# yanyan-li/Structure-SLAM-PointLine

Hardware: AMD Instinct MI355X
Metric: front-end frames/sec (ORB+LSD extract+match) 640x480 @1000kp/200ln (higher is better)
Workload: dtype u8

## Files before the change

include/sslam_frontend.h:

```cpp
#ifndef SSLAM_FRONTEND_H
#define SSLAM_FRONTEND_H

#include <stddef.h>
#include <stdint.h>

#ifdef __cplusplus
extern "C" {
#endif

#define SSLAM_OK 0
#define SSLAM_ERR_INVALID (-1)
#define SSLAM_ERR_NO_DEVICE (-2)
#define SSLAM_ERR_CAPACITY (-3)
#define SSLAM_ERR_HIP (-4)
#define SSLAM_ERR_UNSUPPORTED (-5)

typedef struct sslam_keypoint {
    float x, y, size, angle, response;
    int32_t octave, class_id;
} sslam_keypoint;

typedef struct sslam_keyline {
    float angle;
    int32_t class_id, octave;
// ... 185 lines not shown
int sslam_undistort_keypoints_batch_dev(sslam_ctx* ctx, const sslam_camera* cam, const sslam_keypoint* d_kp, const int32_t* d_counts,
                                        int nframes, int cap, sslam_keypoint* d_kp_un, void* stream);
int sslam_orb_set_camera(sslam_orb* orb, const sslam_camera* cam);
int sslam_frontend_batch_match_camera(sslam_orb* orb, sslam_lines* lines, const sslam_camera* cam, const uint8_t* images, int n, int w, int h,
                                      size_t stride, size_t image_stride, int chunk, sslam_keypoint* kp_out, sslam_keypoint* kpun_out,
                                      uint8_t* desc_out, int32_t* nkp_out, int cap, sslam_keyline* kl_out, uint8_t* ldesc_out,
                                      double* linefn_out, int32_t* nl_out, int lcap, const sslam_batch_match* match);

enum { SSLAM_PIX_GRAY = 0, SSLAM_PIX_RGB = 1, SSLAM_PIX_BGR = 2, SSLAM_PIX_RGBA = 3, SSLAM_PIX_BGRA = 4 };
int sslam_gray_from_color(sslam_ctx* ctx, int format, const uint8_t* img, int w, int h, size_t stride, uint8_t* gray, size_t gray_stride);
int sslam_gray_from_color_batch_dev(sslam_ctx* ctx, int format, const uint8_t* d_src, int w, int h, size_t pitch, size_t image_stride, int nframes,
                                    uint8_t* d_gray, size_t gray_pitch, size_t gray_image_stride, void* stream);
int sslam_frontend_batch_color(sslam_orb* orb, sslam_lines* lines, const sslam_camera* cam, int format, const uint8_t* images, int n, int w, int h,
                               size_t stride, size_t image_stride, int chunk, sslam_keypoint* kp_out, sslam_keypoint* kpun_out, uint8_t* desc_out,
                               int32_t* nkp_out, int cap, sslam_keyline* kl_out, uint8_t* ldesc_out, double* linefn_out, int32_t* nl_out, int lcap,
                               const sslam_batch_match* match);

typedef struct sslam_group sslam_group;
#define SSLAM_GROUP_ID_BYTES 128
typedef struct sslam_record_header { int32_t n_kp, n_ln, frame, bytes; } sslam_record_header;
typedef struct sslam_frontend_params {
    int32_t nfeatures; float scale_factor; int32_t nlevels, ini_th_fast, min_th_fast, max_lines;
} sslam_frontend_params;

int sslam_group_create(int ngpu, sslam_group** out);
int sslam_group_unique_id(uint8_t id_out[SSLAM_GROUP_ID_BYTES]);
int sslam_group_create_rank(int device, int rank, int nranks, const uint8_t id[SSLAM_GROUP_ID_BYTES], sslam_group** out);
int sslam_group_destroy(sslam_group* group);
int sslam_group_size(const sslam_group* group);
int sslam_group_rank(const sslam_group* group);

int sslam_pack_records_dev(sslam_ctx* ctx, int nframes, int frame0, int frame_step,
                           const sslam_keypoint* d_kp, const uint8_t* d_desc, const int32_t* d_nkp, int cap,
                           const sslam_keyline* d_kl, const uint8_t* d_ldesc, const double* d_linefn, const int32_t* d_nl, int lcap,
                           uint8_t* d_out, uint64_t out_capacity, uint64_t* d_total_bytes, void* stream);
uint64_t sslam_record_stream_capacity(int nframes, int cap, int lcap);
int sslam_unpack_records(const uint8_t* stream, uint64_t bytes, int nframes,
                         sslam_keypoint* kp_out, uint8_t* desc_out, int32_t* nkp_out, int cap,
                         sslam_keyline* kl_out, uint8_t* ldesc_out, double* linefn_out, int32_t* nl_out, int lcap, int* nrecords_out);

int sslam_group_gather_dev(sslam_group* group, const uint8_t* d_send, const uint64_t* d_send_bytes,
                           uint8_t* d_recv, uint64_t recv_capacity, uint64_t* bytes_per_rank_out, void* stream);

int sslam_frontend_batch_sharded(sslam_group* group, const sslam_frontend_params* params,
                                 const uint8_t* images, int n, int w, int h, size_t stride, size_t image_stride,
                                 sslam_keypoint* kp_out, uint8_t* desc_out, int32_t* nkp_out, int cap,
                                 sslam_keyline* kl_out, uint8_t* ldesc_out, double* linefn_out, int32_t* nl_out, int lcap);
int sslam_shard_layout(int n, int ngpu, int* chunk_slots_out, int* nchunks_out);
int sslam_shard_frame(int n, int ngpu, int chunk, int gpu, int slot);
int sslam_shard_chunk_count(int n, int ngpu, int chunk, int gpu);

int sslam_lines_debug_segments(sslam_lines* ln, int frame, float* seg_out, int cap, int* n_out);
int sslam_lines_debug_cycles(sslam_lines* ln, int frame, long long* out8);
#ifdef __cplusplus
}
#endif
#endif
```

structure-slam-pointline_amd/csrc/lines.hip:

```cpp
#include "common.h"
#include <cmath>
#include <cstdlib>
#include <cfloat>
#include <algorithm>

namespace sslam { int launch_nfa_stream(sslam_ctx* ctx, hipStream_t st, uint8_t* ws, const void* plan, size_t planBytes, const double* lgam, uint8_t* clArea, size_t clFrameBytes,
                                        size_t stageOff, int nframes, int waves, long long spinTicks, bool besideCore); }
namespace sslam { int launch_nfa_stage(sslam_ctx* ctx, hipStream_t st, uint8_t* ws, const void* plan, size_t planBytes, const double* lgam, int nframes); }

using namespace sslam;

namespace {

#include "lsd_plan.h"
#include "lsd_front.h"
#include "lsd_regions.h"
#include "lsd_cluster.h"
#include "lsd_nfa.h"
#include "lbd.h"

__global__ void k_zero_misc(uint8_t* ws, LsdPlan P) {
    Misc* m = (Misc*)(ws + (size_t)blockIdx.x * P.frameBytes + P.offMisc);
    if (threadIdx.x == 0) {
        m->maxS = 0; m->nDefined = 0; m->nSeg = 0; m->nCand = 0; m->nKl = 0; m->overflow = 0; m->claim = 0;
#if defined(SSLAM_LSD_DRIFT_VERIFY) || defined(SSLAM_LSD_CYCLES)
        m->cyc[5] = 0; m->cyc[6] = 0; m->cyc[7] = 0;
#endif
    }
}

__global__ __launch_bounds__(256) void k_lines_status(const uint8_t* __restrict__ ws, LsdPlan P, int nframes, int maxLines, int cap, int* __restrict__ status) {
    __shared__ int cnt[2], first[2];
    if (threadIdx.x < 2) { cnt[threadIdx.x] = 0; first[threadIdx.x] = 0x7FFFFFFF; }
    __syncthreads();
    for (int b = threadIdx.x; b < nframes; b += 256) {
        const Misc* m = (const Misc*)(ws + (size_t)b * P.frameBytes + P.offMisc);
        if (min(m->nSeg, maxLines) > cap) { atomicAdd(&cnt[0], 1); atomicMin(&first[0], b); }
        if (m->overflow) { atomicAdd(&cnt[1], 1); atomicMin(&first[1], b); }
    }
    __syncthreads();
    if (threadIdx.x == 0) { status[0] = cnt[0]; status[1] = first[0]; status[2] = cnt[1]; status[3] = first[1]; }
}

}

struct sslam_lines {
    sslam_ctx* ctx;
    int maxLines;
    int planW = 0, planH = 0;
    LsdPlan plan;
    DevBuf dWs, dTabs, dTaps, dLgam, dGtab;
    size_t clFrame = 0; int clSlots = 0;
    DevBuf dCl;
    int wsFrames = 0, lastFrames = 0;
    hipEvent_t coreEvent = nullptr;
    hipEvent_t coreWait = nullptr, coreDone = nullptr;
    int lastN = -1;
    DevBuf dImg, dKl, dDesc, dFn, dCounts;
    HostPinned hOut;
    bool constsUploaded = false;
    int blurVariant = 0;
    int nfaVariant = 1, lbdBitOrder = 1, lsdResize = 0;
    int seedOrder = 0;
    int sMin = 0;
    bool fusedGeometry = false;
    hipStream_t nfaStream = nullptr; hipEvent_t nfaFork = nullptr, nfaJoin = nullptr;
};

static std::vector<int> taps_q8(int n, double sigma) {
    std::vector<double> k(n);
    double sum = 0, s2 = -0.5 / (sigma * sigma);
    for (int i = 0; i < n; ++i) { double x = i - (n - 1) * 0.5; k[i] = std::exp(s2 * x * x); sum += k[i]; }
    std::vector<int> t(n);
    double err = 0; long isum = 0;
    for (int i = 0; i < n / 2; ++i) {
        double adj = k[i] / sum * 256.0 + err;
        int v = (int)lrint(adj);
        err = adj - v; t[i] = t[n - 1 - i] = v; isum += v;
    }
// ... 484 lines not shown
    std::lock_guard<std::recursive_mutex> lk(L->ctx->mu);
    int rc;
    if ((rc = L->dCounts.ensure(16))) return rc;
    hipStream_t st = stream_ ? (hipStream_t)stream_ : L->ctx->stream;
    if ((rc = sslam_lines_batch_status_dev(L, cap, L->dCounts.as<int32_t>(), st))) return rc;
    int h[4] = {0, 0, 0, 0};
    SSLAM_HIP(hipMemcpyAsync(h, L->dCounts.p, sizeof(h), hipMemcpyDeviceToHost, st));
    SSLAM_HIP(hipStreamSynchronize(st));
    if (truncated_frames_out) *truncated_frames_out = h[0];
    if (unsupported_frames_out) *unsupported_frames_out = h[2];
    if (first_frame_out) *first_frame_out = h[2] ? h[3] : h[0] ? h[1] : -1;
    if (h[2]) { set_error("sslam_lines_batch_status: %d frame(s) with more than %d candidate rectangles (first: frame %d)", h[2], MAX_SEG, h[3]); return SSLAM_ERR_UNSUPPORTED; }
    if (h[0]) { set_error("sslam_lines_batch_status: %d frame(s) hold more lines than the capacity %d (first: frame %d)", h[0], cap, h[1]); return SSLAM_ERR_CAPACITY; }
    return SSLAM_OK;
}

extern "C" int sslam_lines_debug_segments(sslam_lines* L, int frame, float* seg_out, int cap, int* n_out) {
    if (!L || frame < 0 || frame >= L->lastFrames || !n_out) return SSLAM_ERR_INVALID;
    SSLAM_HIP(hipSetDevice(L->ctx->device));
    SSLAM_HIP(hipStreamSynchronize(L->ctx->stream));
    const LsdPlan& P = L->plan;
    const uint8_t* base = L->dWs.as<uint8_t>() + (size_t)frame * P.frameBytes;
    Misc m;
    SSLAM_HIP(hipMemcpy(&m, base + P.offMisc, sizeof(m), hipMemcpyDeviceToHost));
    *n_out = m.nSeg;
    int n = std::min(m.nSeg, cap);
    if (n > 0 && seg_out) SSLAM_HIP(hipMemcpy(seg_out, base + P.offSeg, sizeof(float) * 4 * (size_t)n, hipMemcpyDeviceToHost));
    return SSLAM_OK;
}

extern "C" int sslam_lines_set_core_event(sslam_lines* L, void* hip_event) {
    if (!L) return SSLAM_ERR_INVALID;
    L->coreEvent = (hipEvent_t)hip_event;
    return SSLAM_OK;
}

extern "C" int sslam_lines_set_core_gate(sslam_lines* L, void* wait_event, void* done_event) {
    if (!L) return SSLAM_ERR_INVALID;
    L->coreWait = (hipEvent_t)wait_event; L->coreDone = (hipEvent_t)done_event;
    return SSLAM_OK;
}

extern "C" int sslam_lines_debug_cycles(sslam_lines* L, int frame, long long* out8) {
    if (!L || frame < 0 || frame >= L->lastFrames || !out8) return SSLAM_ERR_INVALID;
    SSLAM_HIP(hipSetDevice(L->ctx->device));
    SSLAM_HIP(hipDeviceSynchronize());
    const LsdPlan& P = L->plan;
    Misc m;
    SSLAM_HIP(hipMemcpy(&m, L->dWs.as<uint8_t>() + (size_t)frame * P.frameBytes + P.offMisc, sizeof(m), hipMemcpyDeviceToHost));
    for (int i = 0; i < 8; ++i) out8[i] = m.cyc[i];
    return SSLAM_OK;
}

#ifdef SSLAM_TESTING
extern "C" int sslam_lines_debug_cluster(sslam_lines* L, int frame, long long* out8) {
    if (!L || frame < 0 || frame >= L->clSlots || !out8 || !L->dCl.p || !L->clFrame) return SSLAM_ERR_INVALID;
    SSLAM_HIP(hipSetDevice(L->ctx->device));
    SSLAM_HIP(hipDeviceSynchronize());
    ClCtl c;
    SSLAM_HIP(hipMemcpy(&c, L->dCl.as<uint8_t>() + (size_t)frame * L->clFrame, sizeof(c), hipMemcpyDeviceToHost));
    for (int i = 0; i < 8; ++i) out8[i] = c.stat[i];
    return SSLAM_OK;
}

namespace {
struct ScopedDev {
    void* p = nullptr;
    ~ScopedDev() { if (p) (void)hipFree(p); }
};
}

extern "C" int sslam_selftest_exact_div(sslam_ctx* ctx, int n, long long pairs, long long* mismatches_out) {
    if (!ctx || n < 3 || pairs <= 0 || !mismatches_out) return SSLAM_ERR_INVALID;
    SSLAM_HIP(hipSetDevice(ctx->device));
    ScopedDev tabMem, badMem;
    SSLAM_HIP(hipMalloc(&tabMem.p, sizeof(double) * (2 * (size_t)n + 48)));
    SSLAM_HIP(hipMalloc(&badMem.p, sizeof(unsigned long long)));
    double* tab = (double*)tabMem.p; unsigned long long* bad = (unsigned long long*)badMem.p;
    SSLAM_HIP(hipMemset(bad, 0, sizeof(unsigned long long)));
    { const int rc = upload_nfa_tables(tab, n, ctx->stream); if (rc) return rc; }
    const int threads = 256 * 1024, iters = (int)((pairs + threads - 1) / threads);
    hipLaunchKernelGGL(k_selftest_div, dim3(1024), dim3(256), 0, ctx->stream, tab + n + 48, n, 0x1234567ull, iters, bad);
    unsigned long long h = 0;
    SSLAM_HIP(hipMemcpyAsync(&h, bad, sizeof(h), hipMemcpyDeviceToHost, ctx->stream));
    SSLAM_HIP(hipStreamSynchronize(ctx->stream));
    *mismatches_out = (long long)h;
    return SSLAM_OK;
}

extern "C" int sslam_selftest_tail_test(sslam_ctx* ctx, long long samples, long long* disagree_out, long long* ambiguous_out) {
    if (!ctx || samples <= 0 || !disagree_out || !ambiguous_out) return SSLAM_ERR_INVALID;
    SSLAM_HIP(hipSetDevice(ctx->device));
    ScopedDev dMem;
    SSLAM_HIP(hipMalloc(&dMem.p, 2 * sizeof(unsigned long long)));
    unsigned long long* d = (unsigned long long*)dMem.p;
    SSLAM_HIP(hipMemset(d, 0, 2 * sizeof(unsigned long long)));
    const int threads = 256 * 1024, iters = (int)((samples + threads - 1) / threads);
    const double logNT = 5 * (std::log10(512.0) + std::log10(384.0)) / 2 + std::log10(11.0);
    hipLaunchKernelGGL(k_selftest_tail, dim3(1024), dim3(256), 0, ctx->stream, 0xABCDEF12345ull, iters, logNT, d);
    unsigned long long h[2] = {0, 0};
    SSLAM_HIP(hipMemcpyAsync(h, d, sizeof(h), hipMemcpyDeviceToHost, ctx->stream));
    SSLAM_HIP(hipStreamSynchronize(ctx->stream));
    *disagree_out = (long long)h[0]; *ambiguous_out = (long long)h[1];
    return SSLAM_OK;
}

// ... 191 lines not shown
```

structure-slam-pointline_amd/csrc/lsd_plan.h:

```cpp
#pragma once

constexpr double kPI = 3.14159265358979323846;
constexpr double DEG2RAD = kPI / 180;
constexpr double M_3_2_PI_ = (3 * kPI) / 2, M_2PI_ = 2 * kPI;
constexpr float NOTDEF_F = -1024.0f;
constexpr int CS_SHIFT = 3, S_SHIFT = 2;
constexpr unsigned USED_BIT = 0x80000000u;
constexpr int N_BINS = 1024;
#ifndef SSLAM_TILE_PX
#define SSLAM_TILE_PX 8192
#endif
constexpr int TILE_PX = SSLAM_TILE_PX;
constexpr int MAX_SEG = 8192;
constexpr int NUM_BANDS = 9, BAND_W = 7, LSP_H = 63;

struct LsdPlan {
    int w, h;
    int sw, sh, spitch;
    int npx;
    int nTiles, tileRows;
    int nXB;
    int sMin;
    size_t frameBytes;
    int tW, cW;
    size_t offBlur, offT, offS, offCs, offCand, offFlag, offNfa, offOrder, offTileHist, offReg, offSeg, offMisc, offDxy, offKl, offSortIdx, offSegCnt, offComp, offSorted, offLbdDir;
    int blurTaps[7];
    int blur5Taps[5];
    int tabX, tabY;
    double rho, prec, p, logNT;
    int minRegSize;
    int nfaVariant;
    int lbdBitOrder;
    int lsdResize;
};

struct Misc {
    int maxS;
    int nDefined;
    int nSeg;
    int nCand;
    int nKl;
    int overflow;
    int claim;
    int pad_;
    long long cyc[8];
};

struct NfaStreamCtl {
    int candReady;
    int candFinal;
    int claim;
    int expired;
};
constexpr int NFA_STREAM_BLOCK = 8;
constexpr int NFA_STREAM_CTL_OFF = 256;

__device__ __forceinline__ int tix(int x, int y, int tW) { return y * tW + x; }
__device__ __forceinline__ int cix(int x, int y, int cW) { return y * cW + x; }

struct RectD { double x1, y1, x2, y2, width, x, y, theta, dx, dy, prec, p; };

#ifndef SSLAM_LSD_QCAP
#define SSLAM_LSD_QCAP 768
#endif
constexpr int QCAP = SSLAM_LSD_QCAP;
constexpr int MAXC = 5;

__device__ __forceinline__ double angle_diff_signed(double a, double b) {
    double diff = a - b;
    while (diff <= -kPI) diff += M_2PI_;
    while (diff > kPI) diff -= M_2PI_;
    return diff;
}
__device__ __forceinline__ bool is_aligned_val(float aDeg, double theta, double prec) {
    double n_theta = fabs(theta - (double)aDeg * DEG2RAD);
    const double wrapped = fabs(n_theta - M_2PI_);
    n_theta = n_theta > M_3_2_PI_ ? wrapped : n_theta;
    return aDeg != NOTDEF_F && n_theta <= prec;
}
```

structure-slam-pointline_amd/csrc/lsd_regions.h:

```cpp
#pragma once

struct RegQ {
    unsigned* lds; unsigned* glb;
    __device__ __forceinline__ unsigned get(int i) const { return i < QCAP ? lds[i] : glb[i]; }
    __device__ __forceinline__ unsigned get_n(int i, int n) const {
        if (n <= QCAP) { unsigned v = lds[i]; asm volatile("" : "+v"(v)); return v; }
        return get(i);
    }
    __device__ __forceinline__ void set(int i, unsigned v) const { if (i < QCAP) lds[i] = v; else glb[i] = v; }
};
struct Planes {
    float* T; const float2* Cs; const int* S; int tW, cW;
    __device__ __forceinline__ unsigned* Tb() const { return (unsigned*)T; }
    __device__ __forceinline__ float ldT(int i) const { return *(const float*)((const char*)T + ((unsigned)i << 2)); }
    __device__ __forceinline__ void stT(int i, float v) const { *(float*)((char*)T + ((unsigned)i << 2)) = v; }
    __device__ __forceinline__ float2 ldCs(int i) const { return *(const float2*)((const char*)Cs + ((unsigned)i << CS_SHIFT)); }
    __device__ __forceinline__ int ti(int x, int y) const { return (int)(__umul24((unsigned)y, (unsigned)tW) + (unsigned)x); }
    __device__ __forceinline__ int ti(unsigned e) const { return (int)(__umul24(e >> 16, (unsigned)tW) + (e & 0xFFFFu)); }

};
__device__ __forceinline__ bool t_free(float t) { return __float_as_int(t) >= 0; }
__device__ __forceinline__ float t_used(float t) { return __int_as_float(__float_as_int(t) | (int)USED_BIT); }
constexpr int MW_BM_WORDS = 256 * 256 / 32, MW_REACH = 126;
__device__ __forceinline__ int mw_bit(int x, int y) { return ((y & 255) << 8) | (x & 255); }
// ... 12 lines not shown
__device__ __forceinline__ double readlane_d(double v, int l) {
    int lo = __builtin_amdgcn_readlane(__double2loint(v), l), hi = __builtin_amdgcn_readlane(__double2hiint(v), l);
    return __hiloint2double(hi, lo);
}

__device__ __forceinline__ float div_unit_range(float a, float b) {
    float r = __builtin_amdgcn_rcpf(b);
    r = __builtin_fmaf(__builtin_fmaf(-b, r, 1.0f), r, r);
    float q = a * r;
    q = __builtin_fmaf(__builtin_fmaf(-b, q, a), r, q);
    return __builtin_fmaf(__builtin_fmaf(-b, q, a), r, q);
}

__device__ __forceinline__ float fast_atan2_deg_unit(float y, float x) {
    const float p1 = 0.9997878412794807f * (float)(180 / 3.14159265358979323846);
    const float p3 = -0.3258083974640975f * (float)(180 / 3.14159265358979323846);
    const float p5 = 0.1555786518463281f * (float)(180 / 3.14159265358979323846);
    const float p7 = -0.04432655554792128f * (float)(180 / 3.14159265358979323846);
    const float eps = (float)2.2204460492503131e-16;
    const float ax = fabsf(x), ay = fabsf(y);
    const float c = div_unit_range(fminf(ax, ay), __fadd_rn(fmaxf(ax, ay), eps));
    const float c2 = __fmul_rn(c, c);
    float a = __fmul_rn(__fadd_rn(__fmul_rn(__fadd_rn(__fmul_rn(__fadd_rn(__fmul_rn(p7, c2), p5), c2), p3), c2), p1), c);
    if (ax < ay) a = __fsub_rn(90.f, a);
    a = fabsf(__fsub_rn(__int_as_float((__float_as_int(x) >> 31) & 0x43340000), a));
    a = fabsf(__fsub_rn(__int_as_float((__float_as_int(y) >> 31) & 0x43b40000), a));
    return a;
}

#ifdef SSLAM_TESTING
__global__ void k_selftest_region_div(unsigned long long seed, int iters, unsigned long long* __restrict__ out) {
    unsigned long long x = seed + (blockIdx.x * (unsigned long long)blockDim.x + threadIdx.x) * 0x9E3779B97F4A7C15ull;
    auto rnd = [&]() { x ^= x << 13; x ^= x >> 7; x ^= x << 17; return (float)((double)(x >> 11) * 0x1p-53); };
    unsigned long long bad = 0, bad2 = 0;
    for (int it = 0; it < iters; ++it) {
        const float ex = exp2f(-54.f + 74.f * rnd()), ey = exp2f(-54.f + 74.f * rnd());
        float sx = (1.f + rnd()) * ex, sy = (1.f + rnd()) * ey;
        const int mode = (int)(rnd() * 16.f);
        if (mode == 0) sy = 0.f; else if (mode == 1) sx = sy; else if (mode == 2) sx = 6.123234e-17f * (float)(1 + (int)(rnd() * 4000.f));
        else if (mode == 3) { sx = (float)(int)(rnd() * 100000.f); sy = (float)(int)(rnd() * 100000.f); if (sx == 0.f && sy == 0.f) sx = 1.f; }
        if ((x & 1) && sx != 0.f) sx = -sx;
        if ((x & 2) && sy != 0.f) sy = -sy;
        if (sx == 0.f && sy == 0.f) continue;
        const float eps = (float)2.2204460492503131e-16;
        const float ax = fabsf(sx), ay = fabsf(sy), mn = fminf(ax, ay), mx = __fadd_rn(fmaxf(ax, ay), eps);
        if (__float_as_int(div_unit_range(mn, mx)) != __float_as_int(__fdiv_rn(mn, mx))) ++bad;
        if (__float_as_int(fast_atan2_deg_unit(sy, sx)) != __float_as_int(fast_atan2_deg<false>(sy, sx))) ++bad2;
    }
    if (bad) atomicAdd(out, bad);
    if (bad2) atomicAdd(out + 1, bad2);
}
#endif

#ifndef SSLAM_LSD_DRIFT
#define SSLAM_LSD_DRIFT 1
#endif
template <bool LAT, bool WIDE, int MARK = MARK_MAP, class G = TorusHelper>
__device__ int region_grow_w(int seedX, int seedY, float seedDeg, float seedCos, float seedSin, int sw, int sh, const Planes& pl, const RegQ& rq,
                             double prec, double& regAngleOut, long long* __restrict__ verifyCnt, unsigned* __restrict__ bm = nullptr, int capN = 0) {
#ifndef SSLAM_LSD_READLANE
#define SSLAM_LSD_READLANE 0
#endif
    static_assert(MARK == MARK_MAP || LAT, "private marks are written by the lone-wave flavour only");
    constexpr bool RL = LAT || SSLAM_LSD_READLANE;
    constexpr bool DRIFT = !WIDE && SSLAM_LSD_DRIFT;
    const int lane = threadIdx.x & 63;
    int n = 1;
    double regAngle = (double)seedDeg * DEG2RAD;
    float sumdx = seedCos, sumdy = seedSin;
    if (lane == 0) {
        rq.set(0, (unsigned)seedX | ((unsigned)seedY << 16));
        if (MARK) { const int bi = bm_bit<G>(seedX, seedY); atomicOr(&bm[bi >> 5], 1u << (bi & 31)); } else pl.stT(pl.ti(seedX, seedY), t_used(seedDeg));
    }
    const int g = lane >> 3, k8 = lane & 7;
    const int k = k8 + (k8 >= 4 ? 1 : 0);
    const int dy = k / 3 - 1, dx = k - (k / 3) * 3 - 1;
    const float precDeg = (float)(prec * (180.0 / kPI));
    const float minM = prec <= 0.45 ? 2.5f : 3.0e38f;
    constexpr float DRIFT_K = 1.007f, DRIFT_E = 0.011f, DRIFT_ADD = 2e-5f, DRIFT_SLACK = 0.05f;
    float thetaRef = seedDeg, band = DRIFT_SLACK;
    bool fresh = true;
    int i = 0;
#ifdef SSLAM_LSD_CYCLES
    long long* cycStage = verifyCnt - 1;
#endif
    while (i < n) {
        if (MARK == MARK_SPEC && n + 64 > capN) return -n;
        const int np = min(8, n - i);
        int nidx = -1, xx = 0, yy = 0; float tv = NOTDEF_F; float2 cs = make_float2(0.f, 0.f);
        unsigned long long candM;
#ifdef SSLAM_LSD_CYCLES
        const long long tS0 = __builtin_readcyclecounter();
#endif
        if (LAT) {
            const unsigned e = rq.get_n(min(i + g, n - 1), n);
            xx = (int)(e & 0xFFFF) + dx; yy = (int)(e >> 16) + dy;
            const int cx = min(max(xx, 0), sw - 1), cy = min(max(yy, 0), sh - 1);
            nidx = pl.ti(cx, cy);
            tv = pl.ldT(nidx);
            cs = pl.ldCs(nidx);
            candM = __builtin_amdgcn_ballot_w64(t_free(tv)) & __builtin_amdgcn_ballot_w64((unsigned)xx < (unsigned)sw) &
                    __builtin_amdgcn_ballot_w64((unsigned)yy < (unsigned)sh) & (np == 8 ? ~0ull : ((1ull << (np * 8)) - 1));
            if (MARK) { const int bi = bm_bit<G>(xx, yy); candM &= ~__builtin_amdgcn_ballot_w64((bm_word<G>(bm, bi >> 5) >> (bi & 31)) & 1u); }
        } else {
            bool cand = false;
            if (g < np) {
                const unsigned e = rq.get_n(i + g, n);
                xx = (int)(e & 0xFFFF) + dx; yy = (int)(e >> 16) + dy;
                if (xx >= 0 && yy >= 0 && xx < sw && yy < sh) {
                    nidx = pl.ti(xx, yy);
                    tv = pl.ldT(nidx);
                    cs = pl.ldCs(nidx);
                    cand = t_free(tv);
                }
            }
            candM = __builtin_amdgcn_ballot_w64(cand);
        }
#ifdef SSLAM_LSD_CYCLES
        const long long tS1 = __builtin_readcyclecounter();
#endif
        const int nBefore = n;
        unsigned long long accMask = 0;
        auto aligned_mask = [&]() -> unsigned long long {
            if (WIDE) return __builtin_amdgcn_ballot_w64(is_aligned_val(tv, regAngle, prec));
            const double d = fabs(regAngle - (double)tv * DEG2RAD);
            return __builtin_amdgcn_ballot_w64(d <= prec) | __builtin_amdgcn_ballot_w64(fabs(d - M_2PI_) <= prec);
        };
        unsigned long long live = candM;
        if (!DRIFT) {
            unsigned long long m = aligned_mask() & live;
            while (m) {
                const int sel = __ffsll((long long)m) - 1;
                const int selIdx = RL ? __builtin_amdgcn_readlane(nidx, sel) : __builtin_amdgcn_ds_bpermute(sel << 2, nidx);
                if (LAT) accMask |= 1ull << sel;
                else if (lane == sel) {
                    const unsigned v = (unsigned)xx | ((unsigned)yy << 16);
                    pl.stT(nidx, t_used(tv)); rq.lds[min(n, QCAP)] = v;
                    if (n >= QCAP) rq.glb[n] = v;
                }
                ++n;
                sumdx = __fadd_rn(sumdx, __int_as_float(RL ? __builtin_amdgcn_readlane(__float_as_int(cs.x), sel) : __builtin_amdgcn_ds_bpermute(sel << 2, __float_as_int(cs.x))));
                sumdy = __fadd_rn(sumdy, __int_as_float(RL ? __builtin_amdgcn_readlane(__float_as_int(cs.y), sel) : __builtin_amdgcn_ds_bpermute(sel << 2, __float_as_int(cs.y))));
                regAngle = (double)fast_atan2_deg_unit(sumdy, sumdx) * DEG2RAD;
                candM &= ~__builtin_amdgcn_ballot_w64(nidx == selIdx);
                m = aligned_mask() & candM & (~1ull << sel);
            }
        } else {
            float dc, u; unsigned long long side;
            auto classify = [&]() {
                const float d = fabsf(__fsub_rn(thetaRef, tv));
                dc = fminf(d, __fsub_rn(360.f, d));
                u = fabsf(__fsub_rn(dc, precDeg));
                side = __builtin_amdgcn_ballot_w64(dc <= precDeg);
            };
            classify();
            while (live) {
                const unsigned long long unc = __builtin_amdgcn_ballot_w64(u < band);
                const unsigned long long cm = (side | unc) & live;
#ifdef SSLAM_LSD_DRIFT_VERIFY
                {
                    const double ra = (double)fast_atan2_deg_unit(sumdy, sumdx) * DEG2RAD;
                    const double d = fabs(ra - (double)tv * DEG2RAD);
                    const unsigned long long mx = (__builtin_amdgcn_ballot_w64(d <= prec) | __builtin_amdgcn_ballot_w64(fabs(d - M_2PI_) <= prec)) & live;
                    const int selX = mx ? __ffsll((long long)mx) - 1 : -1, selC = cm ? __ffsll((long long)cm) - 1 : -1;
                    const bool decided = selC < 0 || !((unc >> selC) & 1ull);
                    if (decided && selC != selX && lane == 0 && verifyCnt) atomicAdd((unsigned long long*)verifyCnt, 1ull);
                    if (lane == 0 && verifyCnt) atomicAdd((unsigned long long*)verifyCnt + 1, decided ? 0x100000001ull : 1ull);
                }
#endif
                if (!cm) break;
                int sel = __ffsll((long long)cm) - 1;
                if ((unc >> sel) & 1ull) {
                    if (!fresh) {
                        const float a = fast_atan2_deg_unit(sumdy, sumdx);
                        regAngle = (double)a * DEG2RAD; thetaRef = a; band = DRIFT_SLACK; fresh = true;
                        classify();
                    }
                    const unsigned long long m = aligned_mask() & live;
                    if (!m) break;
                    sel = __ffsll((long long)m) - 1;
                }
                const int selIdx = RL ? __builtin_amdgcn_readlane(nidx, sel) : __builtin_amdgcn_ds_bpermute(sel << 2, nidx);
                if (LAT) accMask |= 1ull << sel;
                else if (lane == sel) {
                    const unsigned v = (unsigned)xx | ((unsigned)yy << 16);
                    pl.stT(nidx, t_used(tv)); rq.lds[min(n, QCAP)] = v;
                    if (n >= QCAP) rq.glb[n] = v;
                }
                ++n;
                const float dcsEarly = __int_as_float(RL ? __builtin_amdgcn_readlane(__float_as_int(dc), sel) : __builtin_amdgcn_ds_bpermute(sel << 2, __float_as_int(dc)));
                sumdx = __fadd_rn(sumdx, __int_as_float(RL ? __builtin_amdgcn_readlane(__float_as_int(cs.x), sel) : __builtin_amdgcn_ds_bpermute(sel << 2, __float_as_int(cs.x))));
                sumdy = __fadd_rn(sumdy, __int_as_float(RL ? __builtin_amdgcn_readlane(__float_as_int(cs.y), sel) : __builtin_amdgcn_ds_bpermute(sel << 2, __float_as_int(cs.y))));
                {
                    const float dcs = dcsEarly;
                    const float M = fmaxf(fabsf(sumdx), fabsf(sumdy));
                    const float aK = __builtin_fmaf(__fadd_rn(dcs, band), DRIFT_K, (DRIFT_E - DRIFT_SLACK) * DRIFT_K);
                    const float r = M < minM ? 1.0e9f : __builtin_amdgcn_rcpf(M);
                    band = __fadd_rn(__builtin_fmaf(aK, r, band), DRIFT_ADD);
                    fresh = false;
                }
                candM &= ~__builtin_amdgcn_ballot_w64(nidx == selIdx);
                live = candM & (~1ull << sel);
            }
        }
        if (LAT && accMask != 0 && ((accMask >> lane) & 1ull)) {
            if (MARK) { const int bi = bm_bit<G>(xx, yy); atomicOr(&bm[bi >> 5], 1u << (bi & 31)); } else pl.stT(nidx, t_used(tv));
            rq.set(nBefore + mbcnt(accMask), (unsigned)xx | ((unsigned)yy << 16));
        }
        if (MARK == MARK_SPEC && __builtin_amdgcn_ballot_w64(((accMask >> lane) & 1ull) && (abs(xx - seedX) > G::REACH || abs(yy - seedY) > G::REACH))) return -n;
#ifdef SSLAM_LSD_CYCLES
        if (verifyCnt) { const long long tS2 = __builtin_readcyclecounter(); cycStage[0] += tS1 - tS0; cycStage[1] += tS2 - tS1; cycStage[2] += 1; }
#endif
        i += np;
    }
    if (DRIFT && !fresh) regAngle = (double)fast_atan2_deg_unit(sumdy, sumdx) * DEG2RAD;
    regAngleOut = regAngle;
    return n;
}

template <bool LAT, int MARK = MARK_MAP, class G = TorusHelper>
__device__ __forceinline__ int region_grow_m(int seedX, int seedY, float seedDeg, float seedCos, float seedSin, int sw, int sh, const Planes& pl, const RegQ& rq,
                                             double prec, double& regAngleOut, long long* __restrict__ verifyCnt, unsigned* __restrict__ bm = nullptr) {
    if (prec < 1.5) return region_grow_w<LAT, false, MARK, G>(seedX, seedY, seedDeg, seedCos, seedSin, sw, sh, pl, rq, prec, regAngleOut, verifyCnt, bm, 0);
    return region_grow_w<LAT, true, MARK, G>(seedX, seedY, seedDeg, seedCos, seedSin, sw, sh, pl, rq, prec, regAngleOut, verifyCnt, bm, 0);
}

struct OrdSum { double acc; };
__device__ __forceinline__ void ordered_sums_add(OrdSum& S, double* __restrict__ red, double v0, double v1, double v2, int cnt, int lane) {
    red[lane] = v0; red[64 + lane] = v1; red[128 + lane] = v2;
    if (lane < 3) {
        const double* src = red + lane * 64;
        double acc = S.acc;
        int j = 0;
        for (; j + 4 <= cnt; j += 4) {
            const double a0 = src[j], a1 = src[j + 1], a2 = src[j + 2], a3 = src[j + 3];
            acc = acc + a0; acc = acc + a1; acc = acc + a2; acc = acc + a3;
        }
        for (; j < cnt; ++j) acc = acc + src[j];
        S.acc = acc;
    }
}
__device__ __forceinline__ double ordered_sums_get(const OrdSum& S, int which) { return readlane_d(S.acc, which); }

__device__ void region2rect_m(const RegQ& rq, int n, int sw, const int* __restrict__ S, double regAngle, double prec, double p, RectD& rec, double* __restrict__ red) {
    const int lane = threadIdx.x & 63;
    OrdSum S1; S1.acc = 0;
    double wgt0 = 0; int px0 = 0, py0 = 0;
    for (int base = 0; base < n; base += 64) {
        const int i = base + lane;
        double fx = 0, fy = 0, wgt = 0;
        if (i < n) {
            const unsigned e = rq.get_n(i, n);
            const int px = e & 0xFFFF, py = e >> 16;
            wgt = sqrt((double)*(const int*)((const char*)S + ((__umul24((unsigned)py, (unsigned)sw) + (unsigned)px) << S_SHIFT)) / 4.0);
            fx = (double)px * wgt; fy = (double)py * wgt;
            if (base == 0) { wgt0 = wgt; px0 = px; py0 = py; }
        }
        ordered_sums_add(S1, red, fx, fy, wgt, min(64, n - base), lane);
    }
    double x = ordered_sums_get(S1, 0), y = ordered_sums_get(S1, 1);
    const double sum = ordered_sums_get(S1, 2);
    x /= sum; y /= sum;
    OrdSum S2; S2.acc = 0;
    for (int base = 0; base < n; base += 64) {
        const int i = base + lane;
        double a = 0, b = 0, c = 0;
        if (i < n) {
            int px = px0, py = py0; double wgt = wgt0;
            if (base != 0) {
                const unsigned e = rq.get_n(i, n);
                px = e & 0xFFFF; py = e >> 16;
                wgt = sqrt((double)*(const int*)((const char*)S + ((__umul24((unsigned)py, (unsigned)sw) + (unsigned)px) << S_SHIFT)) / 4.0);
            }
            const double ddx = (double)px - x, ddy = (double)py - y;
            a = ddy * ddy * wgt; b = ddx * ddx * wgt; c = ddx * ddy * wgt;
        }
        ordered_sums_add(S2, red, a, b, -c, min(64, n - base), lane);
// ... 159 lines not shown
        sl->nB = n; sl->free += n; sl->cap -= n;
    } else n = region_grow_m<LAT, MARK, G>(x0, y0, sd.x, sd.y, sd.z, sw, sh, pl, rq, tau, regAngle, verifyCnt, MARK ? sl->bm : nullptr);
    if (WANTBOX) {
        unsigned l2, h2;
        if (n <= QCAP) { list_bbox(rq.lds, n, lane, l2, h2); evLo = pk_min_u16(evLo, l2); evHi = pk_max_u16(evHi, h2); } else { evLo = 0u; evHi = 0xFFFFFFFFu; }
    }
    if (n < 2) return false;
    region2rect_m(rq, n, sw, pl.S, regAngle, prec, p, rec, red);
    density = (double)n / (dist_d(rec.x1, rec.y1, rec.x2, rec.y2) * rec.width);
    if (density < DENSITY_TH) {
        const long long tr0 = SSLAM_CLK();
        if (MARK == MARK_SPEC) {
            if (sl->cap < n) {
                for (int i = lane; i < n; i += 64) { const unsigned e = rq.lds[i]; const int bi = bm_bit<G>((int)(e & 0xFFFF), (int)(e >> 16)); atomicAnd(&sl->bm[bi >> 5], ~(1u << (bi & 31))); }
                sl->gaveUp = true; return false;
            }
            for (int i = lane; i < n; i += 64) sl->free[i] = rq.lds[i];
            rq.lds = sl->free; sl->reduced = true;
        }
        const double r1 = (rec.x1 - xc) * (rec.x1 - xc) + (rec.y1 - yc) * (rec.y1 - yc);
        const double r2 = (rec.x2 - xc) * (rec.x2 - xc) + (rec.y2 - yc) * (rec.y2 - yc);
        double radSq = r1 > r2 ? r1 : r2;
        bool good = true;
        while (density < DENSITY_TH) {
            radSq *= 0.75 * 0.75;
            if (MARK == MARK_SPEC) n = remove_far_points_lds<MARK_SPEC, G>(rq.lds, n, xc, yc, radSq, pl, red, sl->bm);
            else if (n <= QCAP) n = remove_far_points_lds<MARK, G>(rq.lds, n, xc, yc, radSq, pl, red, MARK ? sl->bm : nullptr);
            else for (int i = 0; i < n; ++i) {
                const unsigned e = rq.get(i);
                const int px = e & 0xFFFF, py = e >> 16;
                const double d2 = ((double)px - xc) * ((double)px - xc) + ((double)py - yc) * ((double)py - yc);
                if (d2 > radSq) {
                    const unsigned last = rq.get(n - 1);
                    if (lane == 0) {
                        if (MARK) { const int bi = bm_bit<G>(px, py); atomicAnd(&sl->bm[bi >> 5], ~(1u << (bi & 31))); }
                        else { unsigned* t = pl.Tb() + pl.ti(px, py); *t &= ~USED_BIT; }
                        rq.set(i, last);
                    }
                    __builtin_amdgcn_fence(__ATOMIC_SEQ_CST, "workgroup");
                    --n; --i;
                }
            }
            if (n < 2) { good = false; break; }
            region2rect_m(rq, n, sw, pl.S, regAngle, prec, p, rec, red);
            density = (double)n / (dist_d(rec.x1, rec.y1, rec.x2, rec.y2) * rec.width);
        }
        cycs[2] = SSLAM_CLK() - tr0;
        if (!good) return false;
    }
    return true;
}

template <bool LAT>
__device__ __forceinline__ void lsd_regions_body(uint8_t* __restrict__ ws, const LsdPlan& P, int b, unsigned* __restrict__ dynLds, double* __restrict__ red, float4* __restrict__ seedStash) {
    const int lane = threadIdx.x & 63;
    uint8_t* base = ws + (size_t)b * P.frameBytes;
    Planes pl; pl.T = (float*)(base + P.offT); pl.Cs = (const float2*)(base + P.offCs); pl.S = (const int*)(base + P.offS); pl.tW = P.tW; pl.cW = P.cW;
    const unsigned* order = (const unsigned*)(base + P.offOrder);
    double* candOut = (double*)(base + P.offCand);
    Misc* misc = (Misc*)(base + P.offMisc);
    const int sw = P.sw, sh = P.sh;
    RegQ rq; rq.lds = dynLds; rq.glb = (unsigned*)(base + P.offReg);
    const int nOrd = misc->nDefined;
    const double prec = P.prec;
    int nSeg = 0;
    long long cyc0 = 0, cyc1 = 0, cyc2 = 0, cyc3 = 0;
    const long long tStart = SSLAM_CLK();
    for (int pos0 = 0; pos0 < nOrd; pos0 += 64) {
        const int q = pos0 + lane;
        const bool have = q < nOrd;
        const unsigned idx = have ? order[q] : 0xFFFFFFFFu;
        const int tiSeed = have ? pl.ti(idx) : 0;
        const float a0 = have ? pl.ldT(tiSeed) : NOTDEF_F;
        unsigned long long unM = __ballot(t_free(a0));
        if (!unM) continue;
        {
            const double ar = (double)a0 * DEG2RAD;
            seedStash[lane] = make_float4(a0, (float)cos(ar), (float)sin(ar), __int_as_float((int)idx));
        }
        while (unM) {
            const int first = __ffsll((long long)unM) - 1;
            unM &= unM - 1;
            const float4 sd = seedStash[first];
            double regAngle;
            long long t0 = SSLAM_CLK();
            const int sxy = __float_as_int(sd.w), sx = sxy & 0xFFFF, sy = sxy >> 16;
            int n = region_grow_m<LAT>(sx, sy, sd.x, sd.y, sd.z, sw, sh, pl, rq, prec, regAngle, &misc->cyc[6]);
            long long t1 = SSLAM_CLK(); cyc0 += t1 - t0;
            if (n < P.minRegSize) {
                for (int k = 1; k < n; ++k) {
                    const unsigned e = rq.lds[k];
                    unM &= ~__ballot(idx == e);
                }
                continue;
            }
            RectD rec;
            bool refined = false; unsigned evLo = 0xFFFFFFFFu, evHi = 0u;
            long long cycs[3] = {0, 0, 0};
            const int nGrown = n;
            const bool emit = rect_refine<LAT, false, true>(P, sd, n, regAngle, rq, pl, red, rec, refined, evLo, evHi, cycs, nullptr, &misc->cyc[6]);
            cyc1 += cycs[0]; const long long t2 = t1 + cycs[0]; cyc3 += cycs[2];
            if (!refined) { if (nGrown <= QCAP) list_bbox(rq.lds, nGrown, lane, evLo, evHi); else { evLo = 0u; evHi = 0xFFFFFFFFu; } }
            long long t3 = SSLAM_CLK(); cyc2 += t3 - t2;
            {
                const int ix = (int)(idx & 0xFFFF), iy = (int)(idx >> 16);
                const bool chk = have && ((unM >> lane) & 1ull) && ix >= (int)(evLo & 0xFFFF) && ix <= (int)(evHi & 0xFFFF) && iy >= (int)(evLo >> 16) && iy <= (int)(evHi >> 16);
                bool usedNow = false;
                if (chk) usedNow = !t_free(pl.T[tiSeed]);
                unM &= ~__ballot(usedNow);
            }
            if (!emit) continue;
            if (nSeg < MAX_SEG && lane == 0) {
                double* o = candOut + (size_t)nSeg * 12;
                o[0] = rec.x1; o[1] = rec.y1; o[2] = rec.x2; o[3] = rec.y2; o[4] = rec.width; o[5] = rec.x; o[6] = rec.y;
                o[7] = rec.theta; o[8] = rec.dx; o[9] = rec.dy; o[10] = rec.prec; o[11] = rec.p;
            }
            ++nSeg;
        }
    }
    if (lane == 0) {
        misc->nCand = min(nSeg, MAX_SEG); if (nSeg > MAX_SEG) misc->overflow = 1;
        misc->cyc[0] = cyc0; misc->cyc[1] = cyc1; misc->cyc[2] = cyc2; misc->cyc[3] = cyc3; misc->cyc[4] = SSLAM_CLK() - tStart;
    }
}

template <bool LAT, int MW>
__global__ __launch_bounds__(64, MW) void k_lsd_regions(uint8_t* __restrict__ ws, LsdPlan P, const double* __restrict__ lgam, int nframes) {
    extern __shared__ __align__(16) unsigned dynLds[];
    __shared__ double red[3 * 64];
    __shared__ float4 seedStash[64];
    int* claim = &((Misc*)(ws + P.offMisc))->claim;
    for (int i = blockIdx.x; i < nframes;) {
        lsd_regions_body<LAT>(ws, P, xcd_mix_frame(i, nframes), dynLds, red, seedStash);
        if (gridDim.x >= (unsigned)nframes) break;
        int nxt = 0;
        if (threadIdx.x == 0) nxt = atomicAdd(claim, 1);
        i = (int)gridDim.x + __builtin_amdgcn_readfirstlane(nxt);
    }
}
```

Measured before the change: 81800.

## Prefetch next seed neighborhood and next seed window during LSD region growing

In the non-LAT region-grow path, the next unused seed's 8-neighbour angle/cos-sin values are loaded during the last partially filled step of the current region's growth and stashed in LDS. The first step of the next region then reuses them, and the stash is dropped if the finished region touched that seed. Seed-order indices and seed angles for the following two windows are also loaded ahead and parked in LDS, with a re-read only when stale. The change also raises the launch-bounds occupancy hint from 4 to 5 and adds debug counters. The aim is to hide global-memory latency in the serial seed loop, at the cost of extra LDS, registers and more complex control flow.

```diff
diff --git a/include/sslam_frontend.h b/include/sslam_frontend.h
--- a/include/sslam_frontend.h
+++ b/include/sslam_frontend.h
@@ -261,6 +261,7 @@
 
 int sslam_lines_debug_segments(sslam_lines* ln, int frame, float* seg_out, int cap, int* n_out);
 int sslam_lines_debug_cycles(sslam_lines* ln, int frame, long long* out8);
+int sslam_lines_debug_ahead(sslam_lines* ln, int frame, long long* out4);
 #ifdef __cplusplus
 }
 #endif
diff --git a/structure-slam-pointline_amd/csrc/lines.hip b/structure-slam-pointline_amd/csrc/lines.hip
--- a/structure-slam-pointline_amd/csrc/lines.hip
+++ b/structure-slam-pointline_amd/csrc/lines.hip
@@ -24,7 +24,7 @@
     if (threadIdx.x == 0) {
         m->maxS = 0; m->nDefined = 0; m->nSeg = 0; m->nCand = 0; m->nKl = 0; m->overflow = 0; m->claim = 0;
 #if defined(SSLAM_LSD_DRIFT_VERIFY) || defined(SSLAM_LSD_CYCLES)
-        m->cyc[5] = 0; m->cyc[6] = 0; m->cyc[7] = 0;
+        m->cyc[5] = 0; m->cyc[6] = 0; m->cyc[7] = 0; m->cyc[8] = 0; m->cyc[9] = 0; m->cyc[10] = 0; m->cyc[11] = 0;
 #endif
     }
 }
@@ -615,6 +615,17 @@
     return SSLAM_OK;
 }
 
+extern "C" int sslam_lines_debug_ahead(sslam_lines* L, int frame, long long* out4) {
+    if (!L || frame < 0 || frame >= L->lastFrames || !out4) return SSLAM_ERR_INVALID;
+    SSLAM_HIP(hipSetDevice(L->ctx->device));
+    SSLAM_HIP(hipDeviceSynchronize());
+    const LsdPlan& P = L->plan;
+    Misc m;
+    SSLAM_HIP(hipMemcpy(&m, L->dWs.as<uint8_t>() + (size_t)frame * P.frameBytes + P.offMisc, sizeof(m), hipMemcpyDeviceToHost));
+    for (int i = 0; i < 4; ++i) out4[i] = m.cyc[8 + i];
+    return SSLAM_OK;
+}
+
 #ifdef SSLAM_TESTING
 extern "C" int sslam_lines_debug_cluster(sslam_lines* L, int frame, long long* out8) {
     if (!L || frame < 0 || frame >= L->clSlots || !out8 || !L->dCl.p || !L->clFrame) return SSLAM_ERR_INVALID;
diff --git a/structure-slam-pointline_amd/csrc/lsd_plan.h b/structure-slam-pointline_amd/csrc/lsd_plan.h
--- a/structure-slam-pointline_amd/csrc/lsd_plan.h
+++ b/structure-slam-pointline_amd/csrc/lsd_plan.h
@@ -43,7 +43,7 @@
     int overflow;
     int claim;
     int pad_;
-    long long cyc[8];
+    long long cyc[12];
 };
 
 struct NfaStreamCtl {
diff --git a/structure-slam-pointline_amd/csrc/lsd_regions.h b/structure-slam-pointline_amd/csrc/lsd_regions.h
--- a/structure-slam-pointline_amd/csrc/lsd_regions.h
+++ b/structure-slam-pointline_amd/csrc/lsd_regions.h
@@ -88,18 +88,28 @@
 }
 #endif
 
+struct SeedAhead {
+    float4* stash;
+    unsigned xy;
+    bool want;
+    bool use;
+    bool done;
+};
+
 #ifndef SSLAM_LSD_DRIFT
 #define SSLAM_LSD_DRIFT 1
 #endif
 template <bool LAT, bool WIDE, int MARK = MARK_MAP, class G = TorusHelper>
 __device__ int region_grow_w(int seedX, int seedY, float seedDeg, float seedCos, float seedSin, int sw, int sh, const Planes& pl, const RegQ& rq,
-                             double prec, double& regAngleOut, long long* __restrict__ verifyCnt, unsigned* __restrict__ bm = nullptr, int capN = 0) {
+                             double prec, double& regAngleOut, long long* __restrict__ verifyCnt, unsigned* __restrict__ bm = nullptr, int capN = 0,
+                             SeedAhead* __restrict__ ah = nullptr) {
 #ifndef SSLAM_LSD_READLANE
 #define SSLAM_LSD_READLANE 0
 #endif
     static_assert(MARK == MARK_MAP || LAT, "private marks are written by the lone-wave flavour only");
     constexpr bool RL = LAT || SSLAM_LSD_READLANE;
     constexpr bool DRIFT = !WIDE && SSLAM_LSD_DRIFT;
+    constexpr bool AHEAD = !LAT && MARK == MARK_MAP;
     const int lane = threadIdx.x & 63;
     int n = 1;
     double regAngle = (double)seedDeg * DEG2RAD;
@@ -140,17 +150,33 @@
             if (MARK) { const int bi = bm_bit<G>(xx, yy); candM &= ~__builtin_amdgcn_ballot_w64((bm_word<G>(bm, bi >> 5) >> (bi & 31)) & 1u); }
         } else {
             bool cand = false;
-            if (g < np) {
-                const unsigned e = rq.get_n(i + g, n);
+            const bool feed = AHEAD && ah && i == 0 && ah->use;
+            const bool ride = AHEAD && ah && !feed && ah->want && np < 8;
+            if (feed) {
+                if (g == 0) {
+                    xx = seedX + dx; yy = seedY + dy;
+                    if (xx >= 0 && yy >= 0 && xx < sw && yy < sh) {
+                        nidx = pl.ti(xx, yy);
+                        const float4 v = ah->stash[k8]; tv = v.x; cs = make_float2(v.y, v.z);
+                        cand = t_free(tv);
+                    }
+                }
+            } else if (g < np || (ride && g == 7)) {
+                unsigned e = ride ? ah->xy : 0u;
+                if (g < np) e = rq.get_n(i + g, n);
                 xx = (int)(e & 0xFFFF) + dx; yy = (int)(e >> 16) + dy;
                 if (xx >= 0 && yy >= 0 && xx < sw && yy < sh) {
                     nidx = pl.ti(xx, yy);
                     tv = pl.ldT(nidx);
                     cs = pl.ldCs(nidx);
-                    cand = t_free(tv);
+                    cand = g < np && t_free(tv);
                 }
             }
             candM = __builtin_amdgcn_ballot_w64(cand);
+            if (ride) {
+                if (g == 7) ah->stash[k8] = make_float4(tv, cs.x, cs.y, 0.f);
+                ah->want = false; ah->done = true;
+            }
         }
 #ifdef SSLAM_LSD_CYCLES
         const long long tS1 = __builtin_readcyclecounter();
@@ -256,9 +282,10 @@
 
 template <bool LAT, int MARK = MARK_MAP, class G = TorusHelper>
 __device__ __forceinline__ int region_grow_m(int seedX, int seedY, float seedDeg, float seedCos, float seedSin, int sw, int sh, const Planes& pl, const RegQ& rq,
-                                             double prec, double& regAngleOut, long long* __restrict__ verifyCnt, unsigned* __restrict__ bm = nullptr) {
-    if (prec < 1.5) return region_grow_w<LAT, false, MARK, G>(seedX, seedY, seedDeg, seedCos, seedSin, sw, sh, pl, rq, prec, regAngleOut, verifyCnt, bm, 0);
-    return region_grow_w<LAT, true, MARK, G>(seedX, seedY, seedDeg, seedCos, seedSin, sw, sh, pl, rq, prec, regAngleOut, verifyCnt, bm, 0);
+                                             double prec, double& regAngleOut, long long* __restrict__ verifyCnt, unsigned* __restrict__ bm = nullptr,
+                                             SeedAhead* __restrict__ ah = nullptr) {
+    if (prec < 1.5) return region_grow_w<LAT, false, MARK, G>(seedX, seedY, seedDeg, seedCos, seedSin, sw, sh, pl, rq, prec, regAngleOut, verifyCnt, bm, 0, ah);
+    return region_grow_w<LAT, true, MARK, G>(seedX, seedY, seedDeg, seedCos, seedSin, sw, sh, pl, rq, prec, regAngleOut, verifyCnt, bm, 0, ah);
 }
 
 struct OrdSum { double acc; };
@@ -524,7 +551,8 @@
 }
 
 template <bool LAT>
-__device__ __forceinline__ void lsd_regions_body(uint8_t* __restrict__ ws, const LsdPlan& P, int b, unsigned* __restrict__ dynLds, double* __restrict__ red, float4* __restrict__ seedStash) {
+__device__ __forceinline__ void lsd_regions_body(uint8_t* __restrict__ ws, const LsdPlan& P, int b, unsigned* __restrict__ dynLds, double* __restrict__ red, float4* __restrict__ seedStash,
+                                                 unsigned* __restrict__ aheadPark, float4* __restrict__ winStash) {
     const int lane = threadIdx.x & 63;
     uint8_t* base = ws + (size_t)b * P.frameBytes;
     Planes pl; pl.T = (float*)(base + P.offT); pl.Cs = (const float2*)(base + P.offCs); pl.S = (const int*)(base + P.offS); pl.tW = P.tW; pl.cW = P.cW;
@@ -537,19 +565,58 @@
     const double prec = P.prec;
     int nSeg = 0;
     long long cyc0 = 0, cyc1 = 0, cyc2 = 0, cyc3 = 0;
+#ifdef SSLAM_LSD_CYCLES
+    long long ahUsed = 0, ahDropped = 0, ahSkipped = 0, ahReread = 0;
+#define SSLAM_AH_COUNT(x) (x)
+#else
+#define SSLAM_AH_COUNT(x) ((void)0)
+#endif
     const long long tStart = SSLAM_CLK();
+    unsigned idx = 0xFFFFFFFFu, idxN = 0xFFFFFFFFu;
+    float tEarly = NOTDEF_F;
+    bool tCurrent = true;
+    if (!LAT) {
+        if (lane < nOrd) idx = order[lane];
+        if (64 + lane < nOrd) idxN = order[64 + lane];
+        if (idx != 0xFFFFFFFFu) tEarly = pl.ldT(pl.ti(idx));
+    }
+    SeedAhead ah; ah.stash = winStash; ah.xy = 0u; ah.want = false; ah.use = false; ah.done = false;
     for (int pos0 = 0; pos0 < nOrd; pos0 += 64) {
-        const int q = pos0 + lane;
-        const bool have = q < nOrd;
-        const unsigned idx = have ? order[q] : 0xFFFFFFFFu;
-        const int tiSeed = have ? pl.ti(idx) : 0;
-        const float a0 = have ? pl.ldT(tiSeed) : NOTDEF_F;
-        unsigned long long unM = __ballot(t_free(a0));
-        if (!unM) continue;
+        bool have; int tiSeed; float a0; unsigned long long unM;
+        if (LAT) {
+            const int q = pos0 + lane;
+            have = q < nOrd;
+            idx = have ? order[q] : 0xFFFFFFFFu;
+            tiSeed = have ? pl.ti(idx) : 0;
+            a0 = have ? pl.ldT(tiSeed) : NOTDEF_F;
+            unM = __ballot(t_free(a0));
+            if (!unM) continue;
+        } else {
+            have = idx != 0xFFFFFFFFu;
+            tiSeed = have ? pl.ti(idx) : 0;
+            const int q2 = pos0 + 128 + lane;
+            const unsigned idxNN = q2 < nOrd ? order[q2] : 0xFFFFFFFFu;
+            const float tEarlyN = idxN != 0xFFFFFFFFu ? pl.ldT(pl.ti(idxN)) : NOTDEF_F;
+            a0 = tEarly;
+            unM = __ballot(t_free(a0));
+            if (unM && !tCurrent) {
+                if (t_free(a0)) a0 = pl.ldT(tiSeed);
+                unM = __ballot(t_free(a0));
+                SSLAM_AH_COUNT(++ahReread);
+            }
+            if (!unM) {
+                SSLAM_AH_COUNT(++ahSkipped);
+                idx = idxN; idxN = idxNN; tEarly = tEarlyN; tCurrent = true;
+                continue;
+            }
+            aheadPark[lane] = idxN; aheadPark[64 + lane] = idxNN; aheadPark[128 + lane] = __float_as_uint(tEarlyN);
+            tCurrent = false;
+        }
         {
             const double ar = (double)a0 * DEG2RAD;
             seedStash[lane] = make_float4(a0, (float)cos(ar), (float)sin(ar), __int_as_float((int)idx));
         }
+        int pfLane = -1;
         while (unM) {
             const int first = __ffsll((long long)unM) - 1;
             unM &= unM - 1;
@@ -557,13 +624,25 @@
             double regAngle;
             long long t0 = SSLAM_CLK();
             const int sxy = __float_as_int(sd.w), sx = sxy & 0xFFFF, sy = sxy >> 16;
-            int n = region_grow_m<LAT>(sx, sy, sd.x, sd.y, sd.z, sw, sh, pl, rq, prec, regAngle, &misc->cyc[6]);
+            int nxt = -1;
+            if (!LAT) {
+                ah.use = pfLane == first;
+                SSLAM_AH_COUNT(ahUsed += ah.use); SSLAM_AH_COUNT(ahDropped += (pfLane >= 0 && !ah.use));
+                if (unM) { nxt = __ffsll((long long)unM) - 1; ah.xy = (unsigned)__builtin_amdgcn_readfirstlane(__float_as_int(seedStash[nxt].w)); }
+                ah.want = nxt >= 0; ah.done = false;
+            }
+            int n = region_grow_m<LAT>(sx, sy, sd.x, sd.y, sd.z, sw, sh, pl, rq, prec, regAngle, &misc->cyc[6], nullptr, LAT ? nullptr : &ah);
+            pfLane = (!LAT && ah.done) ? nxt : -1;
             long long t1 = SSLAM_CLK(); cyc0 += t1 - t0;
             if (n < P.minRegSize) {
+                const int nx = (int)(ah.xy & 0xFFFF), ny = (int)(ah.xy >> 16);
+                bool hit = abs(sx - nx) <= 1 && abs(sy - ny) <= 1;
                 for (int k = 1; k < n; ++k) {
                     const unsigned e = rq.lds[k];
                     unM &= ~__ballot(idx == e);
-                }
+                    if (!LAT) { const unsigned es = (unsigned)__builtin_amdgcn_readfirstlane((int)e); hit = hit || (abs((int)(es & 0xFFFF) - nx) <= 1 && abs((int)(es >> 16) - ny) <= 1); }
+                }
+                if (pfLane >= 0 && hit) { pfLane = -1; SSLAM_AH_COUNT(++ahDropped); }
                 continue;
             }
             RectD rec;
@@ -574,6 +653,7 @@
             cyc1 += cycs[0]; const long long t2 = t1 + cycs[0]; cyc3 += cycs[2];
             if (!refined) { if (nGrown <= QCAP) list_bbox(rq.lds, nGrown, lane, evLo, evHi); else { evLo = 0u; evHi = 0xFFFFFFFFu; } }
             long long t3 = SSLAM_CLK(); cyc2 += t3 - t2;
+            if (pfLane >= 0 && boxes_meet(ah.xy, ah.xy, evLo, evHi, 1)) { pfLane = -1; SSLAM_AH_COUNT(++ahDropped); }
             {
                 const int ix = (int)(idx & 0xFFFF), iy = (int)(idx >> 16);
                 const bool chk = have && ((unM >> lane) & 1ull) && ix >= (int)(evLo & 0xFFFF) && ix <= (int)(evHi & 0xFFFF) && iy >= (int)(evLo >> 16) && iy <= (int)(evHi >> 16);
@@ -589,21 +669,28 @@
             }
             ++nSeg;
         }
+        if (!LAT) { idx = aheadPark[lane]; idxN = aheadPark[64 + lane]; tEarly = __uint_as_float(aheadPark[128 + lane]); }
     }
     if (lane == 0) {
         misc->nCand = min(nSeg, MAX_SEG); if (nSeg > MAX_SEG) misc->overflow = 1;
         misc->cyc[0] = cyc0; misc->cyc[1] = cyc1; misc->cyc[2] = cyc2; misc->cyc[3] = cyc3; misc->cyc[4] = SSLAM_CLK() - tStart;
-    }
+#ifdef SSLAM_LSD_CYCLES
+        misc->cyc[8] = ahUsed; misc->cyc[9] = ahDropped; misc->cyc[10] = ahSkipped; misc->cyc[11] = ahReread;
+#endif
+    }
+#undef SSLAM_AH_COUNT
 }
 
 template <bool LAT, int MW>
-__global__ __launch_bounds__(64, MW) void k_lsd_regions(uint8_t* __restrict__ ws, LsdPlan P, const double* __restrict__ lgam, int nframes) {
+__global__ __launch_bounds__(64, (!LAT && MW == 4) ? 5 : MW) void k_lsd_regions(uint8_t* __restrict__ ws, LsdPlan P, const double* __restrict__ lgam, int nframes) {
     extern __shared__ __align__(16) unsigned dynLds[];
     __shared__ double red[3 * 64];
     __shared__ float4 seedStash[64];
+    __shared__ unsigned aheadPark[3 * 64];
+    __shared__ float4 winStash[8];
     int* claim = &((Misc*)(ws + P.offMisc))->claim;
     for (int i = blockIdx.x; i < nframes;) {
-        lsd_regions_body<LAT>(ws, P, xcd_mix_frame(i, nframes), dynLds, red, seedStash);
+        lsd_regions_body<LAT>(ws, P, xcd_mix_frame(i, nframes), dynLds, red, seedStash, aheadPark, winStash);
         if (gridDim.x >= (unsigned)nframes) break;
         int nxt = 0;
         if (threadIdx.x == 0) nxt = atomicAdd(claim, 1);
```

After: 77800. 4.9% lower.
